# WeeFav/Visual-Odometry-GPU

Measured on AMD Instinct MI355X. Metric: ORB detect+describe frames/sec (1241x376, 8 lvls), higher is better.
Workload: dtype u8; 1 GPU; KITTI-shaped 1241x376 u8, 8 levels s=1.2, 1000 features, FAST-9 t=20, NMS 3x3, Harris top-N, blur5 all levels, BRIEF-256; batch=1024 frames/step/GPU resident in HBM (stream A); distinct_resident_batches=2, fast_early_exit=True, pyramid_blur_fused=True, pyramid_top_rows_first=True, pipelined_batches=True

## Files before the change

visual-odometry-gpu_amd/csrc/orbx_api.cpp:

```cpp
#include <hip/hip_runtime.h>

#include <algorithm>
#include <array>
#include <cmath>
#include <cstdio>
#include <cstdlib>
#include <cstring>
#include <new>
#include <string>
#include <vector>

#include "orbx_internal.h"
#include "orbx_tri_math.h"

using namespace orbx_geom;

namespace {

thread_local std::string g_create_error;


struct DevBuf {
  void* p = nullptr;
  size_t bytes = 0;
// ... 92 lines not shown
  int device = 0;
  hipStream_t stream = nullptr;
  std::string err;

  OrbxPlan plan{};
  OrbxPlan plan_max{};
  OrbxTileMap tm_blur{};
  OrbxBandMap bm_fast{};
  TileTable tiles[kTileTables];
  OrbxTopLevels top_levels{};
  DevBuf s_tiles;
  std::vector<OrbxResizeTap> h_taps;
  int plan_w = 0, plan_h = 0;

  uint8_t* d_in = nullptr;
  static constexpr int kGraphs = 16;
  hipGraphExec_t g_exec[kGraphs] = {};
  OrbxGraphKey g_key[kGraphs] = {};
  int g_next = 0;
  int plan_serial = 0;
  OrbxResizeTap* d_taps = nullptr;
  size_t taps_capacity = 0;
  float* d_gauss = nullptr;
  static constexpr int kBlocks = 4;
  Block blocks[kBlocks];
  int blk = 0;
  int host_results = 0;
  int next_lane = 1;
  hipStream_t cstream = nullptr;
  Lane lanes[2];
  int lane = 0;
  bool pipelined = false;
  bool last_two_pass = false;
  hipStream_t last_stream = nullptr;

  DevBuf s_img_a, s_img_b, s_f32, s_u16, s_mask, s_kps, s_f32b, s_desc, s_i32, s_kern;
  DevBuf m_q, m_t, m_idx, m_dist, m_match, m_cnt;
  DevBuf lk_img[2], lk_deriv, lk_io;
  void* lk_host = nullptr;
  size_t lk_host_bytes = 0;
  int lk_w = 0, lk_h = 0, lk_top = -1, lk_win = 0, lk_last = -1;
  int match_pairs = 0;
  long long batch_serial = 0, match_serial = -1;
  long long match_gen = 0, pose_match_gen = -1;
  DevBuf pb_pts, pb_n, pb_out, pb_mask, ph_in, ph_pts, ph_n, ph_out, ph_mask;
  int pose_pairs = 0, pose_cap = 0;
// ... 506 lines not shown
                                 L.d_pyr_blur, c->p.blur_levels == ORBX_BLUR_UPPER ? 1 : 0, c->p.blur_kind));
  }
  if (!two_pass) {
    HIPCHK(c, mark(2, true));
    HIPCHK(c, launch_fast_whole(c, s, n, fp, true));
  }
  ts.split = two_pass;
  c->last_two_pass = two_pass;
  HIPCHK(c, mark(3, true));
  HIPCHK(c, mark(4, false));
  HIPCHK(c, mark(5, false));
  const OutLayout& o = B.layout;
  static const int spread = env_int("ORBX_SELECT_SPREAD", -1);
  HIPCHK(c, orbx_launch_level_select_auto(s, P, n, c->p.select_mode, spread, L.d_mask, final_pyr(c), c->d_gauss,
                                          c->p.harris_window, c->p.harris_k, L.d_lcand, L.d_lcount, L.d_lresp,
                                          L.d_cand, L.d_resp, L.d_cand_count, two_pass ? c->d_feedback + 2 : nullptr));
  HIPCHK(c, mark(6, false));
  if (P.out_cap <= 0)
    HIPCHK(c, hipMemsetAsync(B.d + o.counts, 0, sizeof(int32_t) * (size_t)n, s));
  OrbxHostRecord hr{};
  if (c->host_results && P.out_cap > 0 && B.h_dev)
    hr = OrbxHostRecord{(int32_t*)(B.h_dev + o.counts), (uint32_t*)(B.h_dev + o.kp16), (float*)(B.h_dev + o.angle),
                        (orbx_descriptor*)(B.h_dev + o.desc)};
  HIPCHK(c, orbx_launch_describe(s, P, n, final_pyr(c), c->p.patch_size, L.d_cand_count, L.d_cand, L.d_resp,
                                 (int32_t*)(B.d + o.counts), (orbx_keypoint*)(B.d + o.lkp),
                                 (float*)(B.d + o.resp), (int32_t*)(B.d + o.level),
                                 (orbx_keypoint*)(B.d + o.kp), (uint32_t*)(B.d + o.kp16),
                                 (float*)(B.d + o.angle),
                                 (orbx_descriptor*)(B.d + o.desc), two_pass ? c->d_feedback : nullptr,
                                 two_pass ? const_cast<uint32_t*>(c->h_feedback) : nullptr, &hr));
  HIPCHK(c, mark(7, false));
  return ORBX_OK;
}

void drop_graph(orbx_ctx* c, int i) {
  if (c->g_exec[i]) (void)hipGraphExecDestroy(c->g_exec[i]);
  c->g_exec[i] = nullptr;
}

int run_batch(orbx_ctx* c, const uint8_t* d_frames, int n, int w, int h, int row_stride, size_t frame_stride,
              hipStream_t s, bool may_pipeline = false) {
  if (w != c->learn_w || h != c->learn_h) {
    c->learn_w = w;
    c->learn_h = h;
    for (int l = 0; l < ORBX_MAX_LEVELS; l++) c->need_cur[l] = c->need_prev[l] = 0, c->tile_h_pref[l] = 0;
    for (int i = 2; i < ORBX_FEEDBACK_WORDS; i++) c->h_feedback[i] = 0;
    c->need_batches = 0;
// ... 176 lines not shown
    case ORBX_ERR_UNSUPPORTED:
      return "unsupported parameter combination";
    default:
      return "unknown status";
  }
}

const char* orbx_version(void) { return "liborbx 0.1.0 gfx950"; }

const char* orbx_last_error_string(const orbx_ctx* ctx) { return ctx ? ctx->err.c_str() : g_create_error.c_str(); }

void orbx_destroy(orbx_ctx* c) {
  DeviceGuard _dg(c);
  if (!c) return;
  if (c->stream) (void)hipStreamSynchronize(c->stream);
  if (c->lanes[1].stream) (void)hipStreamSynchronize(c->lanes[1].stream);
  for (int i = 0; i < orbx_ctx::kGraphs; i++) drop_graph(c, i);
  for (Lane& L : c->lanes) {
    free_lane(c, L);
    if (L.ev_pool) (void)hipEventDestroy(L.ev_pool);
  }
  for (TileTable& T : c->tiles)
    if (T.d) (void)hipFree(T.d);
  void* bufs[] = {c->d_in, c->d_taps, c->d_gauss, c->d_feedback};
  for (void* b : bufs)
    if (b) (void)hipFree(b);
  if (c->h_feedback) (void)hipHostFree(const_cast<uint32_t*>(c->h_feedback));
  for (Block& B : c->blocks) {
    if (B.h) (void)hipHostFree(B.h);
    if (B.d) (void)hipFree(B.d);
    if (B.ev_done) (void)hipEventDestroy(B.ev_done);
    if (B.ev_copied) (void)hipEventDestroy(B.ev_copied);
  }
  if (c->cstream) {
    (void)hipStreamSynchronize(c->cstream);
    (void)hipStreamDestroy(c->cstream);
  }
  DevBuf* sb[] = {&c->s_img_a, &c->s_img_b, &c->s_f32,  &c->s_u16, &c->s_mask, &c->s_kps,   &c->s_f32b, &c->s_desc,
                  &c->s_i32,   &c->s_kern,  &c->s_tiles, &c->m_q,    &c->m_t,   &c->m_idx,  &c->m_dist,  &c->m_match, &c->m_cnt,
                  &c->lk_img[0], &c->lk_img[1], &c->lk_deriv, &c->lk_io, &c->pb_pts, &c->pb_n, &c->pb_out,
                  &c->pb_mask, &c->ph_in, &c->ph_pts, &c->ph_n, &c->ph_out, &c->ph_mask, &c->sb_xyz, &c->sb_valid,
                  &c->sb_mq, &c->sb_mt, &c->sb_n, &c->sb_out, &c->sh_in, &c->sh_xyz, &c->sh_valid, &c->sh_out,
                  &c->ba_off, &c->ba_poses, &c->ba_points, &c->ba_rows, &c->ba_opose, &c->ba_oxy, &c->ba_wp, &c->ba_wo,
                  &c->ba_slot, &c->ba_out, &c->gf_ws, &c->gf_img, &c->gf_res,
                  &c->lkw_ws, &c->lkw_first, &c->lkw_img, &c->lkw_pts, &c->lkw_res};
  if (c->gf_ev) {
    (void)hipEventSynchronize(c->gf_ev);
// ... 80 lines not shown
  CREATE_CHK(hipMemset(c->d_feedback, 0, ORBX_FEEDBACK_WORDS * 4));
  CREATE_CHK(hipHostMalloc((void**)&c->h_feedback, ORBX_FEEDBACK_WORDS * 4, hipHostMallocDefault));
  for (int i = 0; i < ORBX_FEEDBACK_WORDS; i++) c->h_feedback[i] = 0;
  OrbxTableCapacity tcap{};
  if ((st = table_capacity(*p, M, c->fast_impl, c->blur_impl, &tcap, &why)) != ORBX_OK) {
    orbx_destroy(c);
    return fail(nullptr, st, why);
  }
  for (TileTable& T : c->tiles) T.capacity = tcap.frame;
  c->tiles[T_FAST].capacity = tcap.fast;
  c->tiles[T_PYRBLUR_SMALL].capacity = tcap.small;
  for (TileTable& T : c->tiles)
    CREATE_CHK(hipMalloc((void**)&T.d, std::max<size_t>(T.capacity, 1) * sizeof(OrbxTileDesc)));
  {
    c->taps_capacity = tcap.taps;
    CREATE_CHK(hipMalloc((void**)&c->d_taps, c->taps_capacity * sizeof(OrbxResizeTap)));
  }
  {
    const int K = p->harris_window;
    std::vector<float> g((size_t)K * K);
    gaussian_kernel(K, -1.0f, g.data());
    CREATE_CHK(hipMalloc((void**)&c->d_gauss, g.size() * sizeof(float)));
    CREATE_CHK(hipMemcpy(c->d_gauss, g.data(), g.size() * sizeof(float), hipMemcpyHostToDevice));
  }
  {
    const OutLayout o = make_out_layout((int)B, slots_per_frame(M));
    {
      int least = 0, greatest = 0;
      CREATE_CHK(hipDeviceGetStreamPriorityRange(&least, &greatest));
      CREATE_CHK(hipStreamCreateWithPriority(&c->cstream, hipStreamNonBlocking, greatest));
    }
    for (Block& blk : c->blocks) {
      CREATE_CHK(hipMalloc((void**)&blk.d, o.total));
      CREATE_CHK(hipHostMalloc((void**)&blk.h, o.total, hipHostMallocDefault));
      CREATE_CHK(hipHostGetDevicePointer((void**)&blk.h_dev, blk.h, 0));
      CREATE_CHK(hipEventCreateWithFlags(&blk.ev_done, hipEventDisableTiming));
      CREATE_CHK(hipEventCreateWithFlags(&blk.ev_copied, hipEventDisableTiming));
    }
    for (Lane& L : c->lanes) CREATE_CHK(hipEventCreateWithFlags(&L.ev_pool, hipEventDisableTiming));
  }
#undef CREATE_CHK
  *out = c;
  return ORBX_OK;
}

int orbx_get_plan(orbx_ctx* c, int width, int height, int32_t* level_w, int32_t* level_h, int32_t* quota,
// ... 1914 lines not shown
```

visual-odometry-gpu_amd/csrc/orbx_internal.h:

```cpp
#pragma once
#include <hip/hip_runtime.h>
#include <stdint.h>

#include "../../include/orbx.h"

#include "orbx_plan.h"

__host__ __device__ inline int orbx_mask_x(const OrbxLevel& L, int xw, int b) {
  return L.mask_strip_px ? (xw >> 2) * L.mask_strip_px + (xw & 3) * 64 + b : xw * 64 + b;
}

#define ORBX_FAST_STAT_WORDS (ORBX_MAX_LEVELS * ORBX_MAX_BANDS + ORBX_MAX_LEVELS)
#define ORBX_FEEDBACK_WORDS (2 + ORBX_MAX_LEVELS)
struct OrbxTopLevels {
  int32_t n;
  int32_t stat_index[ORBX_MAX_LEVELS];
  int32_t rows[ORBX_MAX_LEVELS];
  int32_t cap[ORBX_MAX_LEVELS];
};

struct OrbxFastParams {
  int32_t threshold, n, nms_radius;
};

// ... 51 lines not shown
                             int frame_bytes, int mask_words, OrbxFastParams fp, unsigned long long* d_mask,
                             unsigned long long* d_row_stat);
hipError_t orbx_launch_compact(hipStream_t s, const OrbxPlan& plan, int n_frames,
                               const unsigned long long* d_mask, orbx_keypoint* d_cand, int32_t* d_cand_count,
                               int32_t* d_cand_total, int need_total);
hipError_t orbx_launch_harris_flat(hipStream_t s, const uint8_t* d_img, int w, int h, int pitch,
                                   const orbx_keypoint* d_kps, int nkp, const float* d_gauss, int K, float kk,
                                   float* d_resp);
hipError_t orbx_launch_level_select(hipStream_t s, const OrbxPlan& plan, int n_frames, int mode,
                                    const unsigned long long* d_mask, const uint8_t* d_pyr, const float* d_gauss,
                                    int window, float k, orbx_keypoint* d_sel_lkp, float* d_sel_resp,
                                    int32_t* d_sel_count, uint32_t* d_need = nullptr);
hipError_t orbx_launch_level_select_auto(hipStream_t s, const OrbxPlan& plan, int n_frames, int mode, int force,
                                         const unsigned long long* d_mask, const uint8_t* d_pyr,
                                         const float* d_gauss, int window, float k, uint32_t* d_cand,
                                         int32_t* d_ncand, float* d_cresp, orbx_keypoint* d_sel_lkp,
                                         float* d_sel_resp, int32_t* d_sel_count, uint32_t* d_need = nullptr);
struct OrbxHostRecord {
  int32_t* counts;
  uint32_t* kp16;
  float* angle;
  orbx_descriptor* desc;
};
hipError_t orbx_launch_describe(hipStream_t s, const OrbxPlan& plan, int n_frames, const uint8_t* d_pyr,
                                int patch_size, const int32_t* d_sel_count, const orbx_keypoint* d_sel_lkp,
                                const float* d_sel_resp, int32_t* d_out_count, orbx_keypoint* d_out_lkp,
                                float* d_out_resp, int32_t* d_out_level, orbx_keypoint* d_out_kp, uint32_t* d_out_kp16,
                                float* d_out_angle, orbx_descriptor* d_out_desc, const uint32_t* d_feedback = nullptr,
                                uint32_t* h_feedback = nullptr, const OrbxHostRecord* host_record = nullptr);

hipError_t orbx_launch_describe_flat(hipStream_t s, const uint8_t* d_img, int w, int h, int pitch,
                                     const orbx_keypoint* d_kps, int nkp, int patch_size, int use_given_angles,
                                     int do_brief, float* d_angles, orbx_descriptor* d_desc);
hipError_t orbx_launch_nms_f32(hipStream_t s, const float* d_scores, int w, int h, int radius, float threshold,
                               unsigned long long* d_mask, int mask_wpr);
hipError_t orbx_launch_conv2d(hipStream_t s, const uint8_t* d_img, int w, int h, int pitch, const float* d_kernel,
                              int K, int reflect_pad, uint8_t* d_dst, int dst_pitch);
hipError_t orbx_launch_select_flat(hipStream_t s, const float* d_resp, int n, int keep, int32_t* d_idx);

hipError_t orbx_launch_knn2(hipStream_t s, int npairs, int max_nq, const orbx_descriptor* d_q, const int32_t* d_qcount,
                            size_t qstride, const orbx_descriptor* d_t, const int32_t* d_tcount, size_t tstride,
                            double ratio, int32_t* d_idx, int32_t* d_dist, int32_t* d_match, size_t ostride);

struct OrbxPosePt {
  double x1, y1, x2, y2;
};
struct OrbxPoseOut {
  double E[9], R[9], t[3];
// ... 49 lines not shown
```

visual-odometry-gpu_amd/csrc/orbx_kernels.hip:

```cpp
#include <hip/hip_runtime.h>

#include <cstdlib>

#include "orbx_internal.h"
#include "orbx_math.h"
#include "orbx_wave.h"

__constant__ __attribute__((aligned(16))) int8_t c_pattern[1024] = {
#include "pattern_31.inc"
};


typedef uint16_t __attribute__((aligned(1))) u16_unaligned;

__device__ __forceinline__ void decode_tile(const OrbxTileMap& tm, int nlevels, int& l, int& tx, int& ty) {
  const int t = blockIdx.x;
  l = 0;
#pragma unroll 1
  for (int i = 1; i < nlevels; i++)
    if (t >= tm.begin[i]) l = i;
  const int local = t - tm.begin[l];
  ty = local / tm.tiles_x[l];
  tx = local - ty * tm.tiles_x[l];
}
// ... 976 lines not shown
                        cx2 > jb.w - 1 || cy2 > jb.h - 1;
      if (!skip) {
        dx1 = min(max(dx1, -18), 18);
        dy1 = min(max(dy1, -18), 18);
        dx2 = min(max(dx2, -18), 18);
        dy2 = min(max(dy2, -18), 18);
        const int s1 = lds.box[(dy1 + 18) * DESC_HP + dx1 + 18 + off];
        const int s2 = lds.box[(dy2 + 18) * DESC_HP + dx2 + 18 + off];
        bit = s1 < s2;
      }
    }
    desc_out[k] = __ballot(bit);
  }
}



#define DESC_NLD ((DESC_ROWS * (DESC_PITCH / 4) + 63) / 64)

struct DescClip {
  int rlo, rhi, clo, chi;
};
__device__ __forceinline__ DescClip desc_clip(const DescJob& jb) {
  const int py0 = jb.y - DESC_R, ax0 = (jb.x - DESC_R) & ~3;
  return {max(-py0, 0), min(jb.h - 1 - py0, DESC_ROWS - 1), max(-ax0, 0), min(jb.pitch - 4 - ax0, DESC_PITCH - 4)};
}
enum { DESC_INSIDE = 0, DESC_TOP = 1, DESC_CLIPPED = 2 };
__device__ __forceinline__ int desc_kind(const DescJob& jb) {
  const int py0 = jb.y - DESC_R, ax0 = (jb.x - DESC_R) & ~3;
  const bool below = py0 + DESC_ROWS <= jb.h, cols = ax0 >= 0 && ax0 + DESC_PITCH <= jb.pitch;
  return below && cols ? (py0 >= 0 ? DESC_INSIDE : DESC_TOP) : DESC_CLIPPED;
}

template <int KIND>
__device__ __forceinline__ void desc_fetch_border(const DescJob& jb, uint32_t base, const int (&rowk)[DESC_NLD],
                                                  const int (&c3)[3], uint32_t (&regs)[DESC_NLD]) {
  const DescClip cl = desc_clip(jb);
  int cb[3];
#pragma unroll
  for (int m = 0; m < 3; m++) cb[m] = KIND == DESC_TOP ? 4 * c3[m] : min(max(4 * c3[m], cl.clo), cl.chi);
#pragma unroll
  for (int k = 0; k < DESC_NLD; k++) {
    const int r = KIND == DESC_TOP ? max(rowk[k], cl.rlo) : min(max(rowk[k], cl.rlo), cl.rhi);
    regs[k] = *reinterpret_cast<const uint32_t*>(
        jb.img + (base + (__umul24((uint32_t)r, (uint32_t)jb.pitch) + (uint32_t)cb[k % 3])));
  }
}

struct DescLds2 {
  uint32_t patch[DESC_ROWS * DESC_PITCH / 4];
  uint16_t hs[DESC_ROWS * DESC_HP];
};

template <class L>
__device__ __forceinline__ void desc_store_patch(L& lds, int lane, const uint32_t (&regs)[DESC_NLD]) {
#pragma unroll
  for (int k = 0; k < DESC_NLD; k++)
    if (lane + 64 * k < DESC_ROWS * (DESC_PITCH / 4)) lds.patch[lane + 64 * k] = regs[k];
}

template <class L>
__device__ __forceinline__ void desc_zero_outside(L& lds, int lane, const DescClip& cl) {
  constexpr int RD = DESC_PITCH / 4;
  for (int i = lane; i < RD * cl.rlo; i += 64) lds.patch[i] = 0;
  for (int i = RD * (cl.rhi + 1) + lane; i < RD * DESC_ROWS; i += 64) lds.patch[i] = 0;
  if (lane < DESC_ROWS) {
    for (int c = 0; c < cl.clo / 4; c++) lds.patch[lane * RD + c] = 0;
    for (int c = cl.chi / 4 + 1; c < RD; c++) lds.patch[lane * RD + c] = 0;
  }
}

#define DESC_TAG 0x8000u
template <class L>
__device__ __forceinline__ void desc_tag_outside(L& lds, int lane, const DescJob& jb, int off) {
  constexpr int RD = DESC_HP / 2;
  const int rlo = min(max(DESC_R - jb.y, 0), DESC_BROWS), rhi = max(min(jb.h + 17 - jb.y, DESC_BROWS - 1), -1);
  const int jlo = min(max(DESC_R + off - jb.x, 0), DESC_HP), jhi = max(min(jb.w + 17 + off - jb.x, DESC_HP - 1), -1);
  uint32_t* t32 = reinterpret_cast<uint32_t*>(lds.hs);
  for (int i = lane; i < RD * rlo; i += 64) t32[i] = DESC_TAG * 0x10001u;
  for (int i = RD * (rhi + 1) + lane; i < RD * DESC_BROWS; i += 64) t32[i] = DESC_TAG * 0x10001u;
  if (lane < DESC_BROWS) {
    for (int j = 0; j < jlo; j++) lds.hs[lane * DESC_HP + j] = DESC_TAG;
    for (int j = jhi + 1; j < DESC_HP; j++) lds.hs[lane * DESC_HP + j] = DESC_TAG;
  }
  wave_lds_sync();
}

__device__ __forceinline__ DescJob desc_job(const OrbxPlan& plan, const uint8_t* pyr, int f, orbx_keypoint kp,
                                            int level) {
  const OrbxLevel& L = plan.L[level];
  DescJob jb;
  jb.img = pyr + (size_t)f * plan.frame_bytes + L.img_off;
  jb.w = L.w;
  jb.h = L.h;
  jb.pitch = L.pitch;
  jb.x = kp.x;
  jb.y = kp.y;
  jb.valid = true;
  return jb;
}
// ... 25 lines not shown
        acc.x = pk_sub(pk_add(acc.x, nw.x), od.x);
        acc.y = pk_sub(pk_add(acc.y, nw.y), od.y);
        q[(i - 1) % 5] = nw;
        bp[i * (DESC_HP / 4)] = acc;
      }
    }
  }
  wave_lds_sync();
}

__device__ __forceinline__ float lround_f(float v) {
  const float t = __builtin_truncf(v);
  const float fr = __fsub_rn(v, t);
  return __fadd_rn(t, __builtin_truncf(__fadd_rn(fr, fr)));
}

typedef float f2_t __attribute__((ext_vector_type(2)));
typedef int i2_t __attribute__((ext_vector_type(2)));
__device__ __forceinline__ i2_t lround_small2(f2_t v) {
  const f2_t h = {0.5f - 0x1p-25f, 0.5f - 0x1p-25f};
  return __builtin_convertvector(v + __builtin_elementwise_copysign(h, v), i2_t);
}

template <int DESC_KPW, int DESC_NW, int DESC_OCC>
__global__ __launch_bounds__(64 * DESC_NW, DESC_OCC) void k_describe2(OrbxPlan plan, const uint8_t* __restrict__ pyr, int patch_size,
                                                   const int32_t* __restrict__ sel_count,
                                                   const orbx_keypoint* __restrict__ sel_lkp,
                                                   const float* __restrict__ sel_resp,
                                                   int32_t* __restrict__ out_count,
                                                   orbx_keypoint* __restrict__ out_lkp,
                                                   float* __restrict__ out_resp,
                                                   int32_t* __restrict__ out_level,
                                                   orbx_keypoint* __restrict__ out_kp,
                                                   uint32_t* __restrict__ out_kp16,
                                                   float* __restrict__ out_angle,
                                                   orbx_descriptor* __restrict__ out_desc,
                                                   const uint32_t* __restrict__ feedback, uint32_t* __restrict__ feedback_host,
                                                   OrbxHostRecord host) {
  constexpr int DESC_KPB = DESC_NW * DESC_KPW;
  static_assert(2 * DESC_KPB <= 64 * DESC_NW, "trig: two threads per keypoint");
  __shared__ __attribute__((aligned(16))) DescLds2 s_lds[DESC_NW];
  __shared__ int s_m[DESC_KPB][2];
  __shared__ float s_cs[DESC_KPB][2];
  __shared__ uint2 s_mw[4 * (DESC_PITCH / 4)];
  __shared__ __attribute__((aligned(16))) uint32_t s_rec_kp[DESC_KPB], s_rec_angle[DESC_KPB], s_rec_desc[DESC_KPB][8];
  const int f = blockIdx.x, grp = blockIdx.y, tid = threadIdx.x, lane = tid & 63;
  const int wave = __builtin_amdgcn_readfirstlane(tid >> 6);
  static_assert(ORBX_MAX_LEVELS <= 64, "one lane per level");
  const int lvl_cnt = lane < plan.nlevels ? sel_count[f * plan.nlevels + lane] : 0;
  const int lvl_end = wave_scan_incl(lvl_cnt);
  const int count = __builtin_amdgcn_readlane(lvl_end, 63);
  if (grp == 0 && tid == 0) {
    out_count[f] = count;
    if (host.counts) host.counts[f] = count;
  }
  if (feedback_host && grp == 0 && f == 0 && tid < ORBX_FEEDBACK_WORDS) feedback_host[tid] = feedback[tid];
  const int slot0 = grp * DESC_KPB;
  if (slot0 >= count) return;
  DescLds2& lds = s_lds[wave];
  const int pr = patch_size / 2;
  if (tid < 4 * (DESC_PITCH / 4)) {
    const int off = tid / (DESC_PITCH / 4), c = tid - off * (DESC_PITCH / 4);
    uint32_t xw = 0, on = 0;
#pragma unroll
    for (int b = 0; b < 4; b++) {
      const int t = 4 * c + b - off - (DESC_R - pr);
      if (t >= 0 && t <= 2 * pr) {
        xw |= (uint32_t)t << (8 * b);
        on |= 1u << (8 * b);
      }
    }
    s_mw[tid] = make_uint2(xw, on);
  }
  int rowk[DESC_NLD], c3[3];
  uint32_t rin = 0;
  {
    int row = lane / (DESC_PITCH / 4), c = lane - row * (DESC_PITCH / 4);
#pragma unroll
    for (int k = 0; k < DESC_NLD; k++) {
      rowk[k] = min(row, DESC_ROWS - 1);
      __builtin_assume(rowk[k] >= 0 && rowk[k] < DESC_ROWS);
      if (k < 3) c3[k] = c;
      if (lane + 64 * k < DESC_ROWS * (DESC_PITCH / 4) && row >= DESC_R - pr && row <= DESC_R + pr) rin |= 1u << k;
      row += 5;
      c += 4;
      if (c >= DESC_PITCH / 4) {
        c -= DESC_PITCH / 4;
        row += 1;
      }
    }
  }
  __syncthreads();
  const size_t fo = (size_t)f * plan.out_cap;

  const int nk = min(DESC_KPW, max(0, count - (slot0 + wave * DESC_KPW)));
  DescJob jobs[DESC_KPW];
  float scale[DESC_KPW];
  uint32_t regs[DESC_KPW][DESC_NLD];
  int offs[DESC_KPW];
#pragma unroll
  for (int j = 0; j < DESC_KPW; j++) {
    const int slot = min(slot0 + wave * DESC_KPW + j, count - 1);
    const int level = __popcll(__ballot(lvl_end <= slot));
    const int lvl_begin = __builtin_amdgcn_readlane(lvl_end - lvl_cnt, level);
    const size_t src = fo + plan.L[level].out_off + (slot - lvl_begin);
    const orbx_keypoint kp = sel_lkp[src];
    jobs[j] = desc_job(plan, pyr, f, kp, level);
    scale[j] = plan.L[level].scale;
    if (j < nk && lane == 0) {
      out_lkp[fo + slot] = kp;
      out_resp[fo + slot] = sel_resp[src];
      out_level[fo + slot] = level;
    }
  }
#pragma unroll
  for (int j = 0; j < DESC_KPW; j++) {
    const DescJob& jb = jobs[j];
    const int py0 = jb.y - DESC_R, ax0 = (jb.x - DESC_R) & ~3;
    offs[j] = jb.x - DESC_R - ax0;
    const uint32_t base = (uint32_t)(py0 * jb.pitch + ax0);
    const int kind = desc_kind(jb);
    if (kind == DESC_INSIDE) {
#pragma unroll
      for (int k = 0; k < DESC_NLD; k++) {
        regs[j][k] = 0;
        if (lane + 64 * k < DESC_ROWS * (DESC_PITCH / 4))
          regs[j][k] = *reinterpret_cast<const uint32_t*>(jb.img + (base + (__umul24((uint32_t)rowk[k], (uint32_t)jb.pitch) + 4u * (uint32_t)c3[k % 3])));
      }
    } else if (kind == DESC_TOP) {
      desc_fetch_border<DESC_TOP>(jb, base, rowk, c3, regs[j]);
    } else {
      desc_fetch_border<DESC_CLIPPED>(jb, base, rowk, c3, regs[j]);
    }
  }

  int pm[2][DESC_KPW];
#pragma unroll
  for (int j = 0; j < DESC_KPW; j++) {
    const DescJob& jb = jobs[j];
    const int off = offs[j];
    pm[0][j] = pm[1][j] = 0;
    if (j < nk && !(jb.x - pr < 0 || jb.x + pr >= jb.w || jb.y - pr < 0 || jb.y + pr >= jb.h)) {
      uint2 mw[3];
#pragma unroll
      for (int m = 0; m < 3; m++) mw[m] = s_mw[off * (DESC_PITCH / 4) + c3[m]];
      uint32_t X = 0, S = 0, M = 0;
#pragma unroll
      for (int k = 0; k < DESC_NLD; k++) {
        const uint32_t z = regs[j][k] & (uint32_t)(-(int32_t)((rin >> k) & 1u));
        X = __builtin_amdgcn_udot4(z, mw[k % 3].x, X, false);
        const uint32_t rs = __builtin_amdgcn_udot4(z, mw[k % 3].y, 0u, false);
        S += rs;
        M += __umul24((uint32_t)rowk[k], rs);
      }
      pm[0][j] = (int)X - __mul24(pr, (int)S);
      pm[1][j] = (int)M - __mul24(DESC_R, (int)S);
    }
  }
  if constexpr (DESC_KPW == 4) {
    int u[2];
#pragma unroll
    for (int i = 0; i < 2; i++) {
      const auto h0 = __builtin_amdgcn_permlane32_swap(pm[i][0], pm[i][1], false, false);
      const auto h1 = __builtin_amdgcn_permlane32_swap(pm[i][2], pm[i][3], false, false);
      const auto r = __builtin_amdgcn_permlane16_swap(h0[0] + h0[1], h1[0] + h1[1], false, false);
      u[i] = row_sum16(r[0] + r[1]);
    }
    if ((lane & 15) == 0) {
      const int q = wave * DESC_KPW + (((lane >> 4) & 1) << 1 | (lane >> 5));
      s_m[q][0] = u[0];
      s_m[q][1] = u[1];
    }
  } else {
#pragma unroll
    for (int j = 0; j < DESC_KPW; j++) {
      const int m10 = wave_sum(pm[0][j]), m01 = wave_sum(pm[1][j]);
      if (lane == 0) {
        s_m[wave * DESC_KPW + j][0] = m10;
        s_m[wave * DESC_KPW + j][1] = m01;
// ... 3 lines not shown
  __syncthreads();
  if (tid < 2 * DESC_KPB && slot0 + (tid >> 1) < count) {
    const int q = tid >> 1, want_sin = tid & 1;
    const float angle = orbx_atan2f((float)s_m[q][1], (float)s_m[q][0]);
    s_cs[q][want_sin] = orbx_sincosf_impl(angle, want_sin ^ 1);
    if (!want_sin) {
      out_angle[fo + slot0 + q] = angle;
      s_rec_angle[q] = __float_as_uint(angle);
    }
  }
  __syncthreads();

  f2_t patx[4], paty[4];
#pragma unroll
  for (int k = 0; k < 4; k++) {
    const int32_t pk = reinterpret_cast<const int32_t*>(c_pattern)[k * 64 + lane];
    patx[k] = f2_t{(float)(int8_t)(pk & 0xff), (float)(int8_t)((pk >> 16) & 0xff)};
    paty[k] = f2_t{(float)(int8_t)((pk >> 8) & 0xff), (float)(int8_t)((pk >> 24) & 0xff)};
  }
#pragma unroll
  for (int j = 0; j < DESC_KPW; j++) {
    if (j < nk) {
      const DescJob& jb = jobs[j];
      const int q = wave * DESC_KPW + j, off = offs[j];
      DescJob jc = jb;
      asm("" : "+s"(jc.x), "+s"(jc.y));
      desc_store_patch(lds, lane, regs[j]);
      if (desc_kind(jc) != DESC_INSIDE) desc_zero_outside(lds, lane, desc_clip(jc));
      wave_lds_sync();
      desc_box_table_fused(lds, lane);
      const float c = s_cs[q][0], s = s_cs[q][1];
      const bool interior = jc.x >= DESC_R && jc.y >= DESC_R && jc.x < jc.w - DESC_R && jc.y < jc.h - DESC_R;
      if (!interior) desc_tag_outside(lds, lane, jc, off);
      u64 d[4];
      const uint16_t* tbl = &lds.hs[18 * DESC_HP + 18 + off];
      auto idx = [&](int x, int y) {
        int i = __mul24(y, DESC_HP) + x;
        asm("" : "+v"(i));
        return i;
      };
      const f2_t C2 = {c, c}, S2 = {s, s};
#pragma unroll
      for (int k = 0; k < 4; k++) {
        const f2_t X = patx[k], Y = paty[k];
        const i2_t rx = lround_small2(C2 * X - S2 * Y), ry = lround_small2(S2 * X + C2 * Y);
        const int s1 = tbl[idx(rx.x, ry.x)], s2 = reinterpret_cast<const int16_t*>(tbl)[idx(rx.y, ry.y)];
        d[k] = __ballot(s1 < s2);
      }
      wave_lds_sync();
      if (lane == 0) {
        const int gx = (int)__fmul_rn((float)jb.x, scale[j]), gy = (int)__fmul_rn((float)jb.y, scale[j]);
        s_rec_kp[q] = (uint32_t)gx | ((uint32_t)gy << 16);
        u64* sd = reinterpret_cast<u64*>(s_rec_desc[q]);
        sd[0] = d[0];
        sd[1] = d[1];
        sd[2] = d[2];
        sd[3] = d[3];
      }
// ... 195 lines not shown

hipError_t orbx_launch_level_select_auto(hipStream_t s, const OrbxPlan& plan, int n_frames, int mode, int force,
                                         const unsigned long long* d_mask, const uint8_t* d_pyr,
                                         const float* d_gauss, int window, float k, uint32_t* d_cand,
                                         int32_t* d_ncand, float* d_cresp, orbx_keypoint* d_sel_lkp,
                                         float* d_sel_resp, int32_t* d_sel_count, uint32_t* d_need) {
  int maxcap = 2;
  for (int l = 0; l < plan.nlevels; l++) maxcap = plan.L[l].cap > maxcap ? plan.L[l].cap : maxcap;
  const bool spread = mode == ORBX_SELECT_HARRIS &&
                      (lvl_slots(plan, plan.nlevels) > LVL_MAX_SLOTS ||
                       (force >= 0 ? force != 0 : maxcap > LVL_THREADS));
  if (!spread)
    return orbx_launch_level_select(s, plan, n_frames, mode, d_mask, d_pyr, d_gauss, window, k, d_sel_lkp,
                                    d_sel_resp, d_sel_count, d_need);
  hipLaunchKernelGGL(k_lvl_compact, dim3(plan.nlevels, n_frames), dim3(256), 0, s, plan, d_mask, d_cand, d_ncand, d_need);
  hipLaunchKernelGGL(k_lvl_harris, dim3((maxcap + 255) / 256, plan.nlevels, n_frames), dim3(256), 0, s, plan, d_pyr,
                     d_gauss, window, k, d_cand, d_ncand, d_cresp);
  const size_t lds = (size_t)((maxcap + 7) & ~7) * 8;
  hipLaunchKernelGGL(k_lvl_rank, dim3((maxcap + RANK_SLICE - 1) / RANK_SLICE, plan.nlevels, n_frames), dim3(256), lds,
                     s, plan, d_cand, d_ncand, d_cresp, d_sel_lkp, d_sel_resp, d_sel_count);
  return ORBX_LAUNCH_CHECK();
}

hipError_t orbx_launch_describe(hipStream_t s, const OrbxPlan& plan, int n_frames, const uint8_t* d_pyr,
                                int patch_size, const int32_t* d_sel_count, const orbx_keypoint* d_sel_lkp,
                                const float* d_sel_resp, int32_t* d_out_count, orbx_keypoint* d_out_lkp,
                                float* d_out_resp, int32_t* d_out_level, orbx_keypoint* d_out_kp, uint32_t* d_out_kp16,
                                float* d_out_angle, orbx_descriptor* d_out_desc, const uint32_t* d_feedback,
                                uint32_t* h_feedback, const OrbxHostRecord* host_record) {
  const OrbxHostRecord host = host_record ? *host_record : OrbxHostRecord{};
  if (plan.out_cap <= 0) return hipSuccess;
  if ((long long)plan.out_cap * n_frames <= 8192) {
    dim3 grid(n_frames, (plan.out_cap + 3) / 4);
    hipLaunchKernelGGL((k_describe2<1, 4, 1>), grid, dim3(256), 0, s, plan, d_pyr, patch_size, d_sel_count, d_sel_lkp,
                       d_sel_resp, d_out_count, d_out_lkp, d_out_resp, d_out_level, d_out_kp, d_out_kp16, d_out_angle, d_out_desc, d_feedback,
                       h_feedback, host);
  } else {
    dim3 grid(n_frames, (plan.out_cap + 15) / 16);
    hipLaunchKernelGGL((k_describe2<4, 4, 6>), grid, dim3(256), 0, s, plan, d_pyr, patch_size, d_sel_count, d_sel_lkp,
                       d_sel_resp, d_out_count, d_out_lkp, d_out_resp, d_out_level, d_out_kp, d_out_kp16, d_out_angle, d_out_desc, d_feedback,
                       h_feedback, host);
  }
  return ORBX_LAUNCH_CHECK();
}

hipError_t orbx_launch_describe_flat(hipStream_t s, const uint8_t* d_img, int w, int h, int pitch,
                                     const orbx_keypoint* d_kps, int nkp, int patch_size, int use_given_angles,
                                     int do_brief, float* d_angles, orbx_descriptor* d_desc) {
  if (nkp <= 0) return hipSuccess;
  hipLaunchKernelGGL(k_describe_flat, dim3((nkp + 3) / 4), dim3(256), 0, s, d_img, w, h, pitch, d_kps, nkp,
                     patch_size, use_given_angles, do_brief, d_angles, d_desc);
  return ORBX_LAUNCH_CHECK();
}

hipError_t orbx_launch_harris_flat(hipStream_t s, const uint8_t* d_img, int w, int h, int pitch,
                                   const orbx_keypoint* d_kps, int nkp, const float* d_gauss, int K, float kk,
                                   float* d_resp) {
  if (nkp <= 0) return hipSuccess;
  hipLaunchKernelGGL(k_harris2_flat, dim3((nkp + 31) / 32), dim3(256), 0, s, d_img, w, h, pitch, d_kps, nkp,
                     d_gauss, K, kk, d_resp);
  return ORBX_LAUNCH_CHECK();
}

hipError_t orbx_launch_nms_f32(hipStream_t s, const float* d_scores, int w, int h, int radius, float threshold,
// ... 34 lines not shown
```

Before: 600,200 frames/s.

## Precompute per-lane describe geometry table and use unaligned patch loads

Moves the per-block moment-weight LDS table and per-lane row/column index math into a host-built per-lane table read from global memory. Patch fetches now start at the exact keypoint column using unaligned dword loads, which removes the per-keypoint alignment offset from the moment and BRIEF lookup paths. The y-moment is folded into a third dot4 with precomputed row weights. A patch_size==31 specialization also skips the row masks for the middle dwords. This removes a __syncthreads and some ALU work in exchange for extra vector-register pressure, unaligned loads, and shift-based masking at clipped borders.

```diff
diff --git a/visual-odometry-gpu_amd/csrc/orbx_api.cpp b/visual-odometry-gpu_amd/csrc/orbx_api.cpp
--- a/visual-odometry-gpu_amd/csrc/orbx_api.cpp
+++ b/visual-odometry-gpu_amd/csrc/orbx_api.cpp
@@ -138,6 +138,7 @@
   OrbxResizeTap* d_taps = nullptr;
   size_t taps_capacity = 0;
   float* d_gauss = nullptr;
+  OrbxDescLanes* d_desc_lanes = nullptr;
   static constexpr int kBlocks = 4;
   Block blocks[kBlocks];
   int blk = 0;
@@ -690,7 +691,7 @@
   if (c->host_results && P.out_cap > 0 && B.h_dev)
     hr = OrbxHostRecord{(int32_t*)(B.h_dev + o.counts), (uint32_t*)(B.h_dev + o.kp16), (float*)(B.h_dev + o.angle),
                         (orbx_descriptor*)(B.h_dev + o.desc)};
-  HIPCHK(c, orbx_launch_describe(s, P, n, final_pyr(c), c->p.patch_size, L.d_cand_count, L.d_cand, L.d_resp,
+  HIPCHK(c, orbx_launch_describe(s, P, n, final_pyr(c), c->p.patch_size, c->d_desc_lanes, L.d_cand_count, L.d_cand, L.d_resp,
                                  (int32_t*)(B.d + o.counts), (orbx_keypoint*)(B.d + o.lkp),
                                  (float*)(B.d + o.resp), (int32_t*)(B.d + o.level),
                                  (orbx_keypoint*)(B.d + o.kp), (uint32_t*)(B.d + o.kp16),
@@ -913,7 +914,7 @@
   }
   for (TileTable& T : c->tiles)
     if (T.d) (void)hipFree(T.d);
-  void* bufs[] = {c->d_in, c->d_taps, c->d_gauss, c->d_feedback};
+  void* bufs[] = {c->d_in, c->d_taps, c->d_gauss, c->d_desc_lanes, c->d_feedback};
   for (void* b : bufs)
     if (b) (void)hipFree(b);
   if (c->h_feedback) (void)hipHostFree(const_cast<uint32_t*>(c->h_feedback));
@@ -1040,6 +1041,12 @@
     gaussian_kernel(K, -1.0f, g.data());
     CREATE_CHK(hipMalloc((void**)&c->d_gauss, g.size() * sizeof(float)));
     CREATE_CHK(hipMemcpy(c->d_gauss, g.data(), g.size() * sizeof(float), hipMemcpyHostToDevice));
+  }
+  {
+    OrbxDescLanes t;
+    orbx_describe_lane_table(p->patch_size, &t);
+    CREATE_CHK(hipMalloc((void**)&c->d_desc_lanes, sizeof(t)));
+    CREATE_CHK(hipMemcpy(c->d_desc_lanes, &t, sizeof(t), hipMemcpyHostToDevice));
   }
   {
     const OutLayout o = make_out_layout((int)B, slots_per_frame(M));
diff --git a/visual-odometry-gpu_amd/csrc/orbx_internal.h b/visual-odometry-gpu_amd/csrc/orbx_internal.h
--- a/visual-odometry-gpu_amd/csrc/orbx_internal.h
+++ b/visual-odometry-gpu_amd/csrc/orbx_internal.h
@@ -97,8 +97,13 @@
   float* angle;
   orbx_descriptor* desc;
 };
+#define ORBX_DESC_LANE_VECS 5
+struct OrbxDescLanes {
+  uint32_t v[ORBX_DESC_LANE_VECS][64][4];
+};
+void orbx_describe_lane_table(int patch_size, OrbxDescLanes* t);
 hipError_t orbx_launch_describe(hipStream_t s, const OrbxPlan& plan, int n_frames, const uint8_t* d_pyr,
-                                int patch_size, const int32_t* d_sel_count, const orbx_keypoint* d_sel_lkp,
+                                int patch_size, const OrbxDescLanes* d_lanes, const int32_t* d_sel_count, const orbx_keypoint* d_sel_lkp,
                                 const float* d_sel_resp, int32_t* d_out_count, orbx_keypoint* d_out_lkp,
                                 float* d_out_resp, int32_t* d_out_level, orbx_keypoint* d_out_kp, uint32_t* d_out_kp16,
                                 float* d_out_angle, orbx_descriptor* d_out_desc, const uint32_t* d_feedback = nullptr,
diff --git a/visual-odometry-gpu_amd/csrc/orbx_kernels.hip b/visual-odometry-gpu_amd/csrc/orbx_kernels.hip
--- a/visual-odometry-gpu_amd/csrc/orbx_kernels.hip
+++ b/visual-odometry-gpu_amd/csrc/orbx_kernels.hip
@@ -1022,28 +1022,35 @@
   int rlo, rhi, clo, chi;
 };
 __device__ __forceinline__ DescClip desc_clip(const DescJob& jb) {
-  const int py0 = jb.y - DESC_R, ax0 = (jb.x - DESC_R) & ~3;
-  return {max(-py0, 0), min(jb.h - 1 - py0, DESC_ROWS - 1), max(-ax0, 0), min(jb.pitch - 4 - ax0, DESC_PITCH - 4)};
+  const int py0 = jb.y - DESC_R, bx0 = jb.x - DESC_R;
+  return {max(-py0, 0), min(jb.h - 1 - py0, DESC_ROWS - 1), max(-bx0, 0), min(jb.pitch - 4 - bx0, DESC_PITCH - 4)};
 }
 enum { DESC_INSIDE = 0, DESC_TOP = 1, DESC_CLIPPED = 2 };
 __device__ __forceinline__ int desc_kind(const DescJob& jb) {
-  const int py0 = jb.y - DESC_R, ax0 = (jb.x - DESC_R) & ~3;
-  const bool below = py0 + DESC_ROWS <= jb.h, cols = ax0 >= 0 && ax0 + DESC_PITCH <= jb.pitch;
+  const int py0 = jb.y - DESC_R, bx0 = jb.x - DESC_R;
+  const bool below = py0 + DESC_ROWS <= jb.h, cols = bx0 >= 0 && bx0 + DESC_PITCH <= jb.pitch;
   return below && cols ? (py0 >= 0 ? DESC_INSIDE : DESC_TOP) : DESC_CLIPPED;
 }
 
 template <int KIND>
 __device__ __forceinline__ void desc_fetch_border(const DescJob& jb, uint32_t base, const int (&rowk)[DESC_NLD],
-                                                  const int (&c3)[3], uint32_t (&regs)[DESC_NLD]) {
+                                                  const int (&cb3)[3], uint32_t (&regs)[DESC_NLD]) {
   const DescClip cl = desc_clip(jb);
   int cb[3];
 #pragma unroll
-  for (int m = 0; m < 3; m++) cb[m] = KIND == DESC_TOP ? 4 * c3[m] : min(max(4 * c3[m], cl.clo), cl.chi);
+  for (int m = 0; m < 3; m++) cb[m] = KIND == DESC_TOP ? cb3[m] : min(max(cb3[m], cl.clo), cl.chi);
 #pragma unroll
   for (int k = 0; k < DESC_NLD; k++) {
     const int r = KIND == DESC_TOP ? max(rowk[k], cl.rlo) : min(max(rowk[k], cl.rlo), cl.rhi);
-    regs[k] = *reinterpret_cast<const uint32_t*>(
+    regs[k] = *reinterpret_cast<const u32_unaligned*>(
         jb.img + (base + (__umul24((uint32_t)r, (uint32_t)jb.pitch) + (uint32_t)cb[k % 3])));
+  }
+  if (KIND == DESC_CLIPPED && (cl.clo > 0 || cl.chi < DESC_PITCH - 4)) {
+#pragma unroll
+    for (int k = 0; k < DESC_NLD; k++) {
+      const int up = 4 * min(max(cl.clo - cb3[k % 3], 0), 4), down = 4 * min(max(cb3[k % 3] - cl.chi, 0), 4);
+      regs[k] = (((regs[k] << up) << up) >> down) >> down;
+    }
   }
 }
 
@@ -1064,18 +1071,14 @@
   constexpr int RD = DESC_PITCH / 4;
   for (int i = lane; i < RD * cl.rlo; i += 64) lds.patch[i] = 0;
   for (int i = RD * (cl.rhi + 1) + lane; i < RD * DESC_ROWS; i += 64) lds.patch[i] = 0;
-  if (lane < DESC_ROWS) {
-    for (int c = 0; c < cl.clo / 4; c++) lds.patch[lane * RD + c] = 0;
-    for (int c = cl.chi / 4 + 1; c < RD; c++) lds.patch[lane * RD + c] = 0;
-  }
 }
 
 #define DESC_TAG 0x8000u
 template <class L>
-__device__ __forceinline__ void desc_tag_outside(L& lds, int lane, const DescJob& jb, int off) {
+__device__ __forceinline__ void desc_tag_outside(L& lds, int lane, const DescJob& jb) {
   constexpr int RD = DESC_HP / 2;
   const int rlo = min(max(DESC_R - jb.y, 0), DESC_BROWS), rhi = max(min(jb.h + 17 - jb.y, DESC_BROWS - 1), -1);
-  const int jlo = min(max(DESC_R + off - jb.x, 0), DESC_HP), jhi = max(min(jb.w + 17 + off - jb.x, DESC_HP - 1), -1);
+  const int jlo = min(max(DESC_R - jb.x, 0), DESC_HP), jhi = max(min(jb.w + 17 - jb.x, DESC_HP - 1), -1);
   uint32_t* t32 = reinterpret_cast<uint32_t*>(lds.hs);
   for (int i = lane; i < RD * rlo; i += 64) t32[i] = DESC_TAG * 0x10001u;
   for (int i = RD * (rhi + 1) + lane; i < RD * DESC_BROWS; i += 64) t32[i] = DESC_TAG * 0x10001u;
@@ -1147,8 +1150,35 @@
   return __builtin_convertvector(v + __builtin_elementwise_copysign(h, v), i2_t);
 }
 
-template <int DESC_KPW, int DESC_NW, int DESC_OCC>
+__device__ __forceinline__ uint4 desc_lane_vec(const OrbxDescLanes* __restrict__ t, int v, int lane) {
+  return *reinterpret_cast<const uint4*>(t->v[v][lane]);
+}
+
+template <bool P31>
+__device__ __forceinline__ void desc_moments(const uint32_t (&regs)[DESC_NLD], const uint4 (&wv)[4], int pr, int& m10,
+                                             int& m01) {
+  static_assert(64 / (DESC_PITCH / 4) >= DESC_R - 15 && (6 * 64 - 1) / (DESC_PITCH / 4) <= DESC_R + 15 &&
+                    (7 * 64) / (DESC_PITCH / 4) > DESC_R + 15,
+                "P31: dwords 1..5 inside the window rows, dword 7 outside");
+  const uint32_t xw[3] = {wv[0].x, wv[0].y, wv[0].z}, on[3] = {wv[0].w, wv[1].x, wv[1].y};
+  const uint32_t yw[DESC_NLD] = {wv[1].z, wv[1].w, wv[2].x, wv[2].y, wv[2].z, wv[2].w, wv[3].x, wv[3].y};
+  const uint32_t rin = wv[3].z;
+  uint32_t X = 0, S = 0, M = 0;
+#pragma unroll
+  for (int k = 0; k < (P31 ? DESC_NLD - 1 : DESC_NLD); k++) {
+    uint32_t z = regs[k];
+    if (!P31 || k == 0 || k == DESC_NLD - 2) z &= (uint32_t)(-(int32_t)((rin >> k) & 1u));
+    X = __builtin_amdgcn_udot4(z, xw[k % 3], X, false);
+    S = __builtin_amdgcn_udot4(z, on[k % 3], S, false);
+    M = __builtin_amdgcn_udot4(z, yw[k], M, false);
+  }
+  m10 = (int)X - __mul24(pr, (int)S);
+  m01 = (int)M - __mul24(DESC_R, (int)S);
+}
+
+template <int DESC_KPW, int DESC_NW, int DESC_OCC, bool P31>
 __global__ __launch_bounds__(64 * DESC_NW, DESC_OCC) void k_describe2(OrbxPlan plan, const uint8_t* __restrict__ pyr, int patch_size,
+                                                   const OrbxDescLanes* __restrict__ lanes,
                                                    const int32_t* __restrict__ sel_count,
                                                    const orbx_keypoint* __restrict__ sel_lkp,
                                                    const float* __restrict__ sel_resp,
@@ -1167,12 +1197,15 @@
   __shared__ __attribute__((aligned(16))) DescLds2 s_lds[DESC_NW];
   __shared__ int s_m[DESC_KPB][2];
   __shared__ float s_cs[DESC_KPB][2];
-  __shared__ uint2 s_mw[4 * (DESC_PITCH / 4)];
   __shared__ __attribute__((aligned(16))) uint32_t s_rec_kp[DESC_KPB], s_rec_angle[DESC_KPB], s_rec_desc[DESC_KPB][8];
   const int f = blockIdx.x, grp = blockIdx.y, tid = threadIdx.x, lane = tid & 63;
   const int wave = __builtin_amdgcn_readfirstlane(tid >> 6);
   static_assert(ORBX_MAX_LEVELS <= 64, "one lane per level");
   const int lvl_cnt = lane < plan.nlevels ? sel_count[f * plan.nlevels + lane] : 0;
+  const uint4 geo = desc_lane_vec(lanes, 0, lane);
+  uint4 wv[4];
+#pragma unroll
+  for (int v = 0; v < 4; v++) wv[v] = desc_lane_vec(lanes, 1 + v, lane);
   const int lvl_end = wave_scan_incl(lvl_cnt);
   const int count = __builtin_amdgcn_readlane(lvl_end, 63);
   if (grp == 0 && tid == 0) {
@@ -1183,46 +1216,23 @@
   const int slot0 = grp * DESC_KPB;
   if (slot0 >= count) return;
   DescLds2& lds = s_lds[wave];
-  const int pr = patch_size / 2;
-  if (tid < 4 * (DESC_PITCH / 4)) {
-    const int off = tid / (DESC_PITCH / 4), c = tid - off * (DESC_PITCH / 4);
-    uint32_t xw = 0, on = 0;
-#pragma unroll
-    for (int b = 0; b < 4; b++) {
-      const int t = 4 * c + b - off - (DESC_R - pr);
-      if (t >= 0 && t <= 2 * pr) {
-        xw |= (uint32_t)t << (8 * b);
-        on |= 1u << (8 * b);
-      }
-    }
-    s_mw[tid] = make_uint2(xw, on);
-  }
-  int rowk[DESC_NLD], c3[3];
-  uint32_t rin = 0;
+  const int pr = P31 ? 15 : patch_size / 2;
+  int rowk[DESC_NLD], cb3[3];
   {
-    int row = lane / (DESC_PITCH / 4), c = lane - row * (DESC_PITCH / 4);
 #pragma unroll
     for (int k = 0; k < DESC_NLD; k++) {
-      rowk[k] = min(row, DESC_ROWS - 1);
+      rowk[k] = (int)(((k < 4 ? geo.x : geo.y) >> (8 * (k & 3))) & 0xffu);
       __builtin_assume(rowk[k] >= 0 && rowk[k] < DESC_ROWS);
-      if (k < 3) c3[k] = c;
-      if (lane + 64 * k < DESC_ROWS * (DESC_PITCH / 4) && row >= DESC_R - pr && row <= DESC_R + pr) rin |= 1u << k;
-      row += 5;
-      c += 4;
-      if (c >= DESC_PITCH / 4) {
-        c -= DESC_PITCH / 4;
-        row += 1;
-      }
-    }
-  }
-  __syncthreads();
+    }
+#pragma unroll
+    for (int m = 0; m < 3; m++) cb3[m] = (int)((geo.z >> (8 * m)) & 0xffu);
+  }
   const size_t fo = (size_t)f * plan.out_cap;
 
   const int nk = min(DESC_KPW, max(0, count - (slot0 + wave * DESC_KPW)));
   DescJob jobs[DESC_KPW];
   float scale[DESC_KPW];
   uint32_t regs[DESC_KPW][DESC_NLD];
-  int offs[DESC_KPW];
 #pragma unroll
   for (int j = 0; j < DESC_KPW; j++) {
     const int slot = min(slot0 + wave * DESC_KPW + j, count - 1);
@@ -1241,21 +1251,16 @@
 #pragma unroll
   for (int j = 0; j < DESC_KPW; j++) {
     const DescJob& jb = jobs[j];
-    const int py0 = jb.y - DESC_R, ax0 = (jb.x - DESC_R) & ~3;
-    offs[j] = jb.x - DESC_R - ax0;
-    const uint32_t base = (uint32_t)(py0 * jb.pitch + ax0);
+    const uint32_t base = (uint32_t)((jb.y - DESC_R) * jb.pitch + (jb.x - DESC_R));
     const int kind = desc_kind(jb);
     if (kind == DESC_INSIDE) {
 #pragma unroll
-      for (int k = 0; k < DESC_NLD; k++) {
-        regs[j][k] = 0;
-        if (lane + 64 * k < DESC_ROWS * (DESC_PITCH / 4))
-          regs[j][k] = *reinterpret_cast<const uint32_t*>(jb.img + (base + (__umul24((uint32_t)rowk[k], (uint32_t)jb.pitch) + 4u * (uint32_t)c3[k % 3])));
-      }
+      for (int k = 0; k < DESC_NLD; k++)
+        regs[j][k] = *reinterpret_cast<const u32_unaligned*>(jb.img + (base + (__umul24((uint32_t)rowk[k], (uint32_t)jb.pitch) + (uint32_t)cb3[k % 3])));
     } else if (kind == DESC_TOP) {
-      desc_fetch_border<DESC_TOP>(jb, base, rowk, c3, regs[j]);
+      desc_fetch_border<DESC_TOP>(jb, base, rowk, cb3, regs[j]);
     } else {
-      desc_fetch_border<DESC_CLIPPED>(jb, base, rowk, c3, regs[j]);
+      desc_fetch_border<DESC_CLIPPED>(jb, base, rowk, cb3, regs[j]);
     }
   }
 
@@ -1263,23 +1268,9 @@
 #pragma unroll
   for (int j = 0; j < DESC_KPW; j++) {
     const DescJob& jb = jobs[j];
-    const int off = offs[j];
     pm[0][j] = pm[1][j] = 0;
     if (j < nk && !(jb.x - pr < 0 || jb.x + pr >= jb.w || jb.y - pr < 0 || jb.y + pr >= jb.h)) {
-      uint2 mw[3];
-#pragma unroll
-      for (int m = 0; m < 3; m++) mw[m] = s_mw[off * (DESC_PITCH / 4) + c3[m]];
-      uint32_t X = 0, S = 0, M = 0;
-#pragma unroll
-      for (int k = 0; k < DESC_NLD; k++) {
-        const uint32_t z = regs[j][k] & (uint32_t)(-(int32_t)((rin >> k) & 1u));
-        X = __builtin_amdgcn_udot4(z, mw[k % 3].x, X, false);
-        const uint32_t rs = __builtin_amdgcn_udot4(z, mw[k % 3].y, 0u, false);
-        S += rs;
-        M += __umul24((uint32_t)rowk[k], rs);
-      }
-      pm[0][j] = (int)X - __mul24(pr, (int)S);
-      pm[1][j] = (int)M - __mul24(DESC_R, (int)S);
+      desc_moments<P31>(regs[j], wv, pr, pm[0][j], pm[1][j]);
     }
   }
   if constexpr (DESC_KPW == 4) {
@@ -1329,7 +1320,7 @@
   for (int j = 0; j < DESC_KPW; j++) {
     if (j < nk) {
       const DescJob& jb = jobs[j];
-      const int q = wave * DESC_KPW + j, off = offs[j];
+      const int q = wave * DESC_KPW + j;
       DescJob jc = jb;
       asm("" : "+s"(jc.x), "+s"(jc.y));
       desc_store_patch(lds, lane, regs[j]);
@@ -1338,9 +1329,9 @@
       desc_box_table_fused(lds, lane);
       const float c = s_cs[q][0], s = s_cs[q][1];
       const bool interior = jc.x >= DESC_R && jc.y >= DESC_R && jc.x < jc.w - DESC_R && jc.y < jc.h - DESC_R;
-      if (!interior) desc_tag_outside(lds, lane, jc, off);
+      if (!interior) desc_tag_outside(lds, lane, jc);
       u64 d[4];
-      const uint16_t* tbl = &lds.hs[18 * DESC_HP + 18 + off];
+      const uint16_t* tbl = &lds.hs[18 * DESC_HP + 18];
       auto idx = [&](int x, int y) {
         int i = __mul24(y, DESC_HP) + x;
         asm("" : "+v"(i));
@@ -1582,24 +1573,67 @@
   return ORBX_LAUNCH_CHECK();
 }
 
+void orbx_describe_lane_table(int patch_size, OrbxDescLanes* t) {
+  constexpr int RD = DESC_PITCH / 4;
+  const int pr = patch_size / 2;
+  uint32_t xw[RD], on[RD];
+  for (int c = 0; c < RD; c++) {
+    xw[c] = on[c] = 0;
+    for (int b = 0; b < 4; b++) {
+      const int x = 4 * c + b - (DESC_R - pr);
+      if (x >= 0 && x <= 2 * pr) {
+        xw[c] |= (uint32_t)x << (8 * b);
+        on[c] |= 1u << (8 * b);
+      }
+    }
+  }
+  for (int lane = 0; lane < 64; lane++) {
+    uint32_t rows[2] = {0, 0}, geo = 0, yw[DESC_NLD];
+    int c3[3];
+    for (int k = 0; k < DESC_NLD; k++) {
+      const int i = lane + 64 * k, row = i / RD, c = i % RD;
+      const bool in = i < DESC_ROWS * RD && row >= DESC_R - pr && row <= DESC_R + pr;
+      if (k < 3) c3[k] = c;
+      rows[k / 4] |= (uint32_t)(row < DESC_ROWS ? row : DESC_ROWS - 1) << (8 * (k % 4));
+      if (in) geo |= 1u << (24 + k);
+      yw[k] = in ? on[c] * (uint32_t)row : 0;
+    }
+    for (int m = 0; m < 3; m++) geo |= (uint32_t)(4 * c3[m]) << (8 * m);
+    const uint32_t v[ORBX_DESC_LANE_VECS][4] = {{rows[0], rows[1], geo, 0},
+                                                {xw[c3[0]], xw[c3[1]], xw[c3[2]], on[c3[0]]},
+                                                {on[c3[1]], on[c3[2]], yw[0], yw[1]},
+                                                {yw[2], yw[3], yw[4], yw[5]},
+                                                {yw[6], yw[7], geo >> 24, 0}};
+    for (int a = 0; a < ORBX_DESC_LANE_VECS; a++)
+      for (int b = 0; b < 4; b++) t->v[a][lane][b] = v[a][b];
+  }
+}
+
 hipError_t orbx_launch_describe(hipStream_t s, const OrbxPlan& plan, int n_frames, const uint8_t* d_pyr,
-                                int patch_size, const int32_t* d_sel_count, const orbx_keypoint* d_sel_lkp,
+                                int patch_size, const OrbxDescLanes* d_lanes, const int32_t* d_sel_count, const orbx_keypoint* d_sel_lkp,
                                 const float* d_sel_resp, int32_t* d_out_count, orbx_keypoint* d_out_lkp,
                                 float* d_out_resp, int32_t* d_out_level, orbx_keypoint* d_out_kp, uint32_t* d_out_kp16,
                                 float* d_out_angle, orbx_descriptor* d_out_desc, const uint32_t* d_feedback,
                                 uint32_t* h_feedback, const OrbxHostRecord* host_record) {
   const OrbxHostRecord host = host_record ? *host_record : OrbxHostRecord{};
   if (plan.out_cap <= 0) return hipSuccess;
+  auto launch = [&](auto kernel, int kpb) {
+    dim3 grid(n_frames, (plan.out_cap + kpb - 1) / kpb);
+    hipLaunchKernelGGL(kernel, grid, dim3(256), 0, s, plan, d_pyr, patch_size, d_lanes, d_sel_count, d_sel_lkp,
+                       d_sel_resp, d_out_count, d_out_lkp, d_out_resp, d_out_level, d_out_kp, d_out_kp16, d_out_angle,
+                       d_out_desc, d_feedback, h_feedback, host);
+  };
+  const bool p31 = patch_size == 31;
   if ((long long)plan.out_cap * n_frames <= 8192) {
-    dim3 grid(n_frames, (plan.out_cap + 3) / 4);
-    hipLaunchKernelGGL((k_describe2<1, 4, 1>), grid, dim3(256), 0, s, plan, d_pyr, patch_size, d_sel_count, d_sel_lkp,
-                       d_sel_resp, d_out_count, d_out_lkp, d_out_resp, d_out_level, d_out_kp, d_out_kp16, d_out_angle, d_out_desc, d_feedback,
-                       h_feedback, host);
+    if (p31)
+      launch(k_describe2<1, 4, 1, true>, 4);
+    else
+      launch(k_describe2<1, 4, 1, false>, 4);
   } else {
-    dim3 grid(n_frames, (plan.out_cap + 15) / 16);
-    hipLaunchKernelGGL((k_describe2<4, 4, 6>), grid, dim3(256), 0, s, plan, d_pyr, patch_size, d_sel_count, d_sel_lkp,
-                       d_sel_resp, d_out_count, d_out_lkp, d_out_resp, d_out_level, d_out_kp, d_out_kp16, d_out_angle, d_out_desc, d_feedback,
-                       h_feedback, host);
+    if (p31)
+      launch(k_describe2<4, 4, 6, true>, 16);
+    else
+      launch(k_describe2<4, 4, 6, false>, 16);
   }
   return ORBX_LAUNCH_CHECK();
 }
```

New measurement: 605,600 frames/s, median of 6. No clear change (+0.9%).
